# LFY1998/IPDM-PyTorch

Measured on AMD Instinct MI355X. Metric: CT slices/s (full proj+img partial-diffusion sample), higher is better.
Workload: dtype f32

## Files before the change

ipdm-pytorch_amd/csrc/common.h:

```cpp
#pragma once
#include <hip/hip_runtime.h>
#include <cstdarg>
#include <cstdio>
#include <cstring>
#include <string>
#include <vector>
#include "../../include/ipdm_hip.h"

namespace ipdm {

void set_error(const char *fmt, ...);

#define IPDM_HIP_CHECK(expr)                                                                   \
    do {                                                                                       \
        hipError_t e_ = (expr);                                                                \
        if (e_ != hipSuccess) {                                                                \
            ipdm::set_error("%s failed: %s (%s:%d)", #expr, hipGetErrorString(e_), __FILE__,  \
                            __LINE__);                                                         \
            return IPDM_ERR_HIP;                                                               \
        }                                                                                      \
    } while (0)

#define IPDM_REQUIRE(cond, ...)                   \
    do {                                          \
        if (!(cond)) {                            \
            ipdm::set_error(__VA_ARGS__);         \
            return IPDM_ERR_INVALID;              \
        }                                         \
    } while (0)

#define IPDM_LAUNCH_CHECK() IPDM_HIP_CHECK(hipGetLastError())

static inline int cdiv(long a, long b) { return (int)((a + b - 1) / b); }
static inline size_t align_up(size_t v, size_t a) { return (v + a - 1) / a * a; }

enum Opt {
    OPT_CONV_NO_UP2,
    OPT_CONV_NO_WUP2,
    OPT_CONV_LEGACY, OPT_CONV1X1_LEGACY, OPT_CONVS2_LEGACY,
    OPT_CONV_NO_DIRECT, OPT_DIRECT_NO_PLANAR, OPT_DIRECT_MAX_CIN, OPT_DIRECT_NO_S2, OPT_DIRECT_NO_SKIP_FUSE,
    OPT_CONV_DBG, OPT_CONV_VEC4_STRICT, OPT_CONV_NO_SPLITK, OPT_CONV_NO_WINO, OPT_WINO_V1, OPT_WINO2_MIN_TILES, OPT_CONV1X1_NO_QUARTER, OPT_CONV_NO_PW, OPT_PW_ITEM, OPT_PW_FORCE,
    OPT_CONV_NM,
    OPT_GN_TWO_STAGE, OPT_GN_UNFUSED,
    OPT_UNET_TRANSPOSE,
    OPT_ATTN_NO_KVSPLIT, OPT_ATTN_LEGACY, OPT_ATTN_NO_ZSEQ,
    OPT_ART_PER_VIEW,
    OPT_CONV_BF16X3,
    OPT_ATTN_EXACT_F32,
    OPT_ATTN_NO_PRESPLIT,
    OPT_ATTN_NO_PIPELINE,
    OPT_COUNT
};
int opt(Opt o);
bool opt_per_call(int o);
const char *opt_name(int o);
void opt_snapshot(int (&dst)[OPT_COUNT]);
int opt_changed_since(const int (&rec)[OPT_COUNT]);
std::vector<int> opt_per_call_values();

int ensure_dynamic_lds(const void *kernel, size_t bytes);
int device_cu_count();

int unet_io_channels(const ipdm_unet *net, int *cin, int *cout);

__device__ inline double wave_sum(double v)
{
#pragma unroll
    for (int o = 32; o > 0; o >>= 1) v += __shfl_down(v, o, 64);
    return v;
}
__device__ inline float wave_sum(float v)
{
#pragma unroll
    for (int o = 32; o > 0; o >>= 1) v += __shfl_down(v, o, 64);
    return v;
}
__device__ inline float wave_max(float v)
{
#pragma unroll
    for (int o = 32; o > 0; o >>= 1) v = fmaxf(v, __shfl_down(v, o, 64));
    return v;
}

}
```

ipdm-pytorch_amd/csrc/common.hip:

```cpp
#include <cctype>
#include <cstdlib>
#include <mutex>
#include <strings.h>
#include <set>
#include <utility>
#include "common.h"

namespace ipdm {
static thread_local char g_err[512] = "";
void set_error(const char *fmt, ...)
{
    va_list ap;
    va_start(ap, fmt);
    vsnprintf(g_err, sizeof(g_err), fmt, ap);
    va_end(ap);
}

namespace {
std::mutex g_attr_mu;
std::set<std::pair<const void *, int>> g_attr_done;
int g_cus[64];
}

namespace {
struct OptDef { const char *name; int def; bool per_call; int lo = 0, hi = 1; };
const OptDef g_opt_def[OPT_COUNT] = {
    {"conv_no_up2", 0, true},
    {"conv_no_wup2", 0, true},
    {"conv_legacy", 0, false}, {"conv1x1_legacy", 0, false}, {"convs2_legacy", 0, false},
    {"conv_no_direct", 0, false}, {"direct_no_planar", 0, false},
    {"direct_max_cin", 160, false, 0, 160},
    {"direct_no_s2", 0, false}, {"direct_no_skip_fuse", 0, true},
    {"conv_dbg", 0, true, 0, 0x3ff}, {"conv_vec4_strict", 0, false}, {"conv_no_splitk", 0, false},
    {"conv_no_wino", 0, true}, {"wino_v1", 0, true}, {"wino2_min_tiles", 192, true, 0, 1 << 24},
    {"conv1x1_no_quarter", 0, true}, {"conv_no_pw", 0, true}, {"pw_item", 0, true, 0, 2}, {"pw_force", 0, true}, {"conv_nm", 0, true, 0, 2},
    {"gn_two_stage", 0, true}, {"gn_unfused", 0, true},
    {"unet_transpose", -1, true, -1, 1},
    {"attn_no_kvsplit", 0, false}, {"attn_legacy", 0, false}, {"attn_no_zseq", 0, true},
    {"art_per_view", 0, true},
    {"conv_bf16x3", 0, true},
    {"attn_exact_f32", 0, true},
    {"attn_no_presplit", 0, true},
    {"attn_no_pipeline", 0, true},
};
bool opt_value_ok(int i, int v)
{
    return v >= g_opt_def[i].lo && v <= g_opt_def[i].hi;
}
std::mutex g_opt_mu;
int g_opt_val[OPT_COUNT];
bool g_opt_init = false;

void opt_init_locked()
{
    if (g_opt_init) return;
    for (int i = 0; i < OPT_COUNT; ++i) {
        char env[64] = "IPDM_";
        size_t n = 5;
        for (const char *c = g_opt_def[i].name; *c && n + 1 < sizeof(env); ++c) env[n++] = (char)toupper((unsigned char)*c);
        env[n] = 0;
        const char *e = getenv(env);
        g_opt_val[i] = g_opt_def[i].def;
        if (e) {
            char *end = nullptr;
            const long v = strtol(e, &end, 10);
            const int want = (end != e) ? (int)v : 1;
            if (opt_value_ok(i, want)) g_opt_val[i] = want;
            else fprintf(stderr, "libipdm_hip: %s=%s is outside the option's range [%d, %d]: ignored\n", env, e, g_opt_def[i].lo, g_opt_def[i].hi);
        }
    }
    g_opt_init = true;
}
}

int opt(Opt o)
{
    std::lock_guard<std::mutex> lk(g_opt_mu);
    opt_init_locked();
    return g_opt_val[o];
}
bool opt_per_call(int o) { return g_opt_def[o].per_call; }
const char *opt_name(int o) { return g_opt_def[o].name; }
void opt_snapshot(int (&dst)[OPT_COUNT])
{
    std::lock_guard<std::mutex> lk(g_opt_mu);
    opt_init_locked();
    for (int i = 0; i < OPT_COUNT; ++i) dst[i] = g_opt_val[i];
}
std::vector<int> opt_per_call_values()
{
    std::lock_guard<std::mutex> lk(g_opt_mu);
    opt_init_locked();
    std::vector<int> v;
    for (int i = 0; i < OPT_COUNT; ++i)
        if (g_opt_def[i].per_call) v.push_back(g_opt_val[i]);
    return v;
}
int opt_changed_since(const int (&rec)[OPT_COUNT])
{
    std::lock_guard<std::mutex> lk(g_opt_mu);
    opt_init_locked();
    for (int i = 0; i < OPT_COUNT; ++i)
        if (!g_opt_def[i].per_call && g_opt_val[i] != rec[i]) return i;
    return -1;
}
static int opt_find(const char *name)
{
    if (!name) return -1;
    if (!strncmp(name, "IPDM_", 5) || !strncmp(name, "ipdm_", 5)) name += 5;
    for (int i = 0; i < OPT_COUNT; ++i)
        if (!strcasecmp(name, g_opt_def[i].name)) return i;
    return -1;
}

int ensure_dynamic_lds(const void *kernel, size_t bytes)
{
    int dev = 0;
    IPDM_HIP_CHECK(hipGetDevice(&dev));
    std::lock_guard<std::mutex> lk(g_attr_mu);
    if (g_attr_done.count({kernel, dev})) return IPDM_OK;
    IPDM_HIP_CHECK(hipFuncSetAttribute(kernel, hipFuncAttributeMaxDynamicSharedMemorySize, (int)bytes));
    g_attr_done.insert({kernel, dev});
    return IPDM_OK;
}

int device_cu_count()
{
    int dev = 0, v = 0;
    if (hipGetDevice(&dev) != hipSuccess || dev < 0 || dev >= 64) return 256;
    std::lock_guard<std::mutex> lk(g_attr_mu);
    if (!g_cus[dev])
        g_cus[dev] = (hipDeviceGetAttribute(&v, hipDeviceAttributeMultiprocessorCount, dev) == hipSuccess && v > 0) ? v : 256;
    return g_cus[dev];
}
}

extern "C" const char *ipdm_last_error(void) { return ipdm::g_err; }
extern "C" int ipdm_abi_version(void) { return IPDM_ABI_VERSION; }

extern "C" int ipdm_set_option(const char *name, int value)
{
    const int i = ipdm::opt_find(name);
    IPDM_REQUIRE(i >= 0, "ipdm_set_option: unknown option '%s'", name ? name : "(null)");
    IPDM_REQUIRE(ipdm::opt_value_ok(i, value), "ipdm_set_option: %s = %d is outside [%d, %d]", ipdm::g_opt_def[i].name, value,
                 ipdm::g_opt_def[i].lo, ipdm::g_opt_def[i].hi);
    std::lock_guard<std::mutex> lk(ipdm::g_opt_mu);
    ipdm::opt_init_locked();
    ipdm::g_opt_val[i] = value;
    return IPDM_OK;
}

extern "C" int ipdm_get_option(const char *name, int *value)
{
    const int i = ipdm::opt_find(name);
    IPDM_REQUIRE(i >= 0 && value, "ipdm_get_option: unknown option '%s'", name ? name : "(null)");
    *value = ipdm::opt((ipdm::Opt)i);
    return IPDM_OK;
}
```

ipdm-pytorch_amd/csrc/conv_direct.hip:

```cpp
#include <cstdlib>
#include <type_traits>
#include "common.h"
#include "unet_kernels.h"

using namespace ipdm;

typedef float f32x2 __attribute__((ext_vector_type(2)));
typedef float f32x4 __attribute__((ext_vector_type(4)));

namespace {

inline double direct_bytes(const ConvArgs &a)
{
    return 4.0 * a.B * ((double)(a.C1 + a.C2 + (a.sk_w ? a.sk_C1 + a.sk_C2 : 0)) * a.Hs * a.Ws + (double)a.Cout * a.Ho * a.Wo * (a.res ? 2 : 1));
}

inline bool direct_compute_bound(const ConvArgs &a) { return a.C1 + a.C2 >= 64; }
inline double direct_flops(const ConvArgs &a, int taps)
{
    return 2.0 * a.B * a.Ho * a.Wo * a.Cout * ((double)(a.C1 + a.C2) * taps + (a.sk_w ? a.sk_C1 + a.sk_C2 : 0));
}
inline int direct_class(const ConvArgs &a) { return direct_compute_bound(a) ? 6 : 4; }
inline double direct_work(const ConvArgs &a, int taps) { return direct_compute_bound(a) ? direct_flops(a, taps) : direct_bytes(a); }

constexpr int DT_W = 64, DT_H = 16;

struct DTile { int bx, by, n; };
__device__ inline DTile direct_tile()
{
    const int gx = gridDim.x, gy = gridDim.y;
    const int total = gx * gy * gridDim.z;
    const int L = blockIdx.x + gx * (blockIdx.y + gy * blockIdx.z);
    const int xcd = L & 7, idx = L >> 3, q = total >> 3, r = total & 7;
    const int t = xcd * q + min(xcd, r) + idx;
    DTile d;
    d.bx = t % gx;
    const int rest = t / gx;
    d.by = rest % gy;
    d.n = rest / gy;
    return d;
}
constexpr int DIN_P1 = 68;

#define IPDM_DPP_F(v, ctrl) __builtin_bit_cast(float, __builtin_amdgcn_update_dpp(0, __builtin_bit_cast(int, (v)), (ctrl), 0xf, 0xf, false))
__device__ inline float sum_lanes_row(float x)
{
    x += IPDM_DPP_F(x, 0x121);
    x += IPDM_DPP_F(x, 0x122);
    x += IPDM_DPP_F(x, 0x124);
    x += IPDM_DPP_F(x, 0x128);
    return x;
}
#undef IPDM_DPP_F

constexpr int DOOB = 0x7fffffff;
__device__ inline float dload(__amdgpu_buffer_rsrc_t r, int voff, int soff)
{
    return __builtin_bit_cast(float, __builtin_amdgcn_raw_buffer_load_b32(r, voff, soff, 0));
}

template <int CO>
__device__ inline void direct_epilogue(const ConvArgs &a, f32x2 (&acc)[4][CO / 2], int n, int ox0, int oy0, int tx, int ty, float *in_lds)
{
    const int tid = threadIdx.x;
    const int oy = oy0 + ty, ox = ox0 + tx * 4;
    const bool in_img = oy < a.Ho && ox < a.Wo;
    const size_t out_plane = (size_t)a.Ho * a.Wo;
    const bool vec = (a.Wo & 3) == 0;
    const bool full_tile = oy0 + DT_H <= a.Ho && ox0 + DT_W <= a.Wo;
    float *st = in_lds;
    if (a.stats) __syncthreads();
#pragma unroll
    for (int co = 0; co < CO; ++co) {
        if (co < a.Cout) {
            const float b = a.bias ? a.bias[co] : 0.0f;
            const size_t o = ((size_t)n * a.Cout + co) * out_plane + (size_t)oy * a.Wo + ox;
            f32x4 v = {acc[0][co / 2][co & 1] + b, acc[1][co / 2][co & 1] + b, acc[2][co / 2][co & 1] + b, acc[3][co / 2][co & 1] + b};
            if (in_img) {
                if (vec) {
                    if (a.res) v += *reinterpret_cast<const f32x4 *>(a.res + o);
                    *reinterpret_cast<f32x4 *>(a.out + o) = v;
                } else {
#pragma unroll
                    for (int p = 0; p < 4; ++p)
                        if (ox + p < a.Wo) {
                            v[p] += a.res ? a.res[o + p] : 0.0f;
                            a.out[o + p] = v[p];
                        }
                }
            }
            if (a.stats) {
                if (!full_tile) {
#pragma unroll
                    for (int p = 0; p < 4; ++p) v[p] = (in_img && ox + p < a.Wo) ? v[p] : 0.0f;
                }
                st[(2 * co) * 256 + tid] = (v[0] + v[1]) + (v[2] + v[3]);
                st[(2 * co + 1) * 256 + tid] = fmaf(v[3], v[3], fmaf(v[2], v[2], fmaf(v[1], v[1], v[0] * v[0])));
            }
        }
    }
    if (a.stats) {
        __syncthreads();
        const int j = tid & 15;
#pragma unroll
        for (int k = tid >> 4; k < 2 * CO; k += 16) {
            if ((k >> 1) < a.Cout) {
                const f32x4 *src = reinterpret_cast<const f32x4 *>(st + k * 256 + j * 16);
                const f32x4 p0 = src[0], p1 = src[1], p2 = src[2], p3 = src[3];
                float s = (((p0[0] + p0[1]) + (p0[2] + p0[3])) + ((p1[0] + p1[1]) + (p1[2] + p1[3]))) +
                          (((p2[0] + p2[1]) + (p2[2] + p2[3])) + ((p3[0] + p3[1]) + (p3[2] + p3[3])));
                s = sum_lanes_row(s);
                if (j == 0) {
                    const int row = (oy0 / DT_H) * gridDim.x + ox0 / DT_W;
                    a.stats[(((size_t)n * a.stats_rows + row) * a.Cout + (k >> 1)) * 2 + (k & 1)] = s;
                }
            }
        }
    }
}

template <int CO, int KS, int DKC, bool PLANAR, int STRIDE = 1, int SKIP = 0>
__global__ void __launch_bounds__(256, (STRIDE == 2 ? (CO <= 8 ? 4 : 3) : (CO <= 4 ? 6 : (CO <= 8 ? 5 : 3)))) conv_direct_kernel(ConvArgs a)
{
    static_assert(SKIP == 0 || (KS == 3 && STRIDE == 1 && !PLANAR), "conv_direct: the fused shortcut rides on a 3x3 stride-1 NCHW layer");
    constexpr int DIN_H = (DT_H - 1) * STRIDE + KS, DIN_W = (DT_W - 1) * STRIDE + KS, DIN_P = STRIDE == 1 ? DIN_P1 : 132;
    constexpr int DIN_CH = DIN_H * DIN_P, TAPS = KS * KS, PAD = KS / 2;
    static_assert(STRIDE == 1 || (KS == 3 && !PLANAR), "conv_direct: stride 2 is the 3x3 Downsample");
    __shared__ __attribute__((aligned(16))) float in_lds[DKC * DIN_CH];
    typedef const __attribute__((address_space(4))) float cfloat;
    cfloat *wk = (cfloat *)(unsigned long long)a.w;
    cfloat *gsc = (cfloat *)(unsigned long long)a.gn_scale, *gsh = (cfloat *)(unsigned long long)a.gn_shift;
    const int tid = threadIdx.x;
    const int tx = tid & 15, ty = tid >> 4;
    const DTile dt = direct_tile();
    const int n = dt.n;
    const int ox0 = dt.bx * DT_W, oy0 = dt.by * DT_H;
    const int Ctot = a.C1 + a.C2;
    const int src_plane = a.Hs * a.Ws;

    f32x2 acc[4][CO / 2];
#pragma unroll
    for (int p = 0; p < 4; ++p)
#pragma unroll
        for (int c = 0; c < CO / 2; ++c) acc[p][c] = f32x2{0.0f, 0.0f};

    constexpr int NSP = (DIN_H * DIN_W + 255) / 256;
    int sp_src[NSP], sp_srcp[NSP], sp_dst[NSP];
    bool sp_ok[NSP];
#pragma unroll
    for (int j = 0; j < NSP; ++j) {
        const int e = tid + j * 256;
        const int r = e / DIN_W, c = e % DIN_W;
        const int iy = oy0 * STRIDE - PAD + r, ix = ox0 * STRIDE - PAD + c;
        sp_ok[j] = e < DIN_H * DIN_W && iy >= 0 && iy < a.H && ix >= 0 && ix < a.W;
        int sy = min(max(iy, 0), a.H - 1), sx = min(max(ix, 0), a.W - 1);
        if (a.upsample) {
            sy = min((int)floorf((float)sy * a.scale_y), a.Hs - 1);
            sx = min((int)floorf((float)sx * a.scale_x), a.Ws - 1);
        }
        sp_src[j] = e < DIN_H * DIN_W ? (sy * a.Ws + sx) * 4 : DOOB;
        sp_srcp[j] = !(PLANAR || SKIP == 2) ? sp_src[j]
                   : (e < DIN_H * DIN_W ? ((((sy & 1) * 2 + (sx & 1)) * (a.Hs >> 1) + (sy >> 1)) * (a.Ws >> 1) + (sx >> 1)) * 4 : DOOB);
        sp_dst[j] = e < DIN_H * DIN_W ? r * DIN_P + c : -1;
    }
    const int plane_bytes = src_plane * 4;
    const __amdgpu_buffer_rsrc_t rsrc1 = __builtin_amdgcn_make_buffer_rsrc((void *)(a.x1 + (size_t)n * a.C1 * src_plane), 0, a.C1 * plane_bytes, 0x00020000);
    const __amdgpu_buffer_rsrc_t rsrc2 = __builtin_amdgcn_make_buffer_rsrc((void *)(a.x2 ? a.x2 + (size_t)n * a.C2 * src_plane : a.x1), 0, a.x2 ? a.C2 * plane_bytes : 0, 0x00020000);

    auto run_chunks = [&](auto sk_tag) __attribute__((always_inline)) {
    constexpr bool SK = decltype(sk_tag)::value;
    const int C1v = SK ? a.sk_C1 : a.C1, Ctotv = SK ? a.sk_C1 + a.sk_C2 : Ctot;
    const int actv = SK ? 0 : a.act;
    const __amdgpu_buffer_rsrc_t rsA = SK ? __builtin_amdgcn_make_buffer_rsrc((void *)(a.sk_x1 + (size_t)n * a.sk_C1 * src_plane), 0, a.sk_C1 * plane_bytes, 0x00020000) : rsrc1;
    const __amdgpu_buffer_rsrc_t rsB = SK ? __builtin_amdgcn_make_buffer_rsrc((void *)(a.sk_x2 ? a.sk_x2 + (size_t)n * a.sk_C2 * src_plane : a.sk_x1), 0,
                                                                               a.sk_x2 ? a.sk_C2 * plane_bytes : 0, 0x00020000) : rsrc2;
    constexpr bool PL = SK ? SKIP == 2 : PLANAR;
    cfloat *wkv = SK ? (cfloat *)(unsigned long long)a.sk_w : wk;
    const int cpadv = SK ? a.sk_cout_pad : a.cout_pad;
    for (int c0 = 0; c0 < Ctotv; c0 += DKC) {
        const int kc = min(DKC, Ctotv - c0);
        __syncthreads();
        float raw[DKC][NSP];
#pragma unroll
        for (int c = 0; c < DKC; ++c) {
            const int cg = min(c0 + c, Ctotv - 1);
            const bool from1 = cg < C1v;
            const __amdgpu_buffer_rsrc_t r = from1 ? rsA : rsB;
            const int so = (from1 ? cg : cg - C1v) * plane_bytes;
#pragma unroll
            for (int j = 0; j < NSP; ++j) raw[c][j] = dload(r, PL && from1 ? sp_srcp[j] : sp_src[j], so);
        }
#pragma unroll
        for (int c = 0; c < DKC; ++c) {
            if (c < kc) {
                float sc = 1.0f, sh = 0.0f;
                if (actv) { sc = gsc[(size_t)n * Ctot + c0 + c]; sh = gsh[(size_t)n * Ctot + c0 + c]; }
#pragma unroll
                for (int j = 0; j < NSP; ++j) {
                    float v = raw[c][j];
                    if (actv) {
                        v = v * sc + sh;
                        if (actv == 2) v = v * __builtin_amdgcn_rcpf(1.0f + __builtin_amdgcn_exp2f(-1.4426950408889634f * v));
                    }
                    if (sp_dst[j] >= 0) in_lds[c * DIN_CH + sp_dst[j]] = sp_ok[j] ? v : 0.0f;
                }
            }
        }
        __syncthreads();
        for (int c = 0; c < kc; ++c) {
            const float *ip = in_lds + c * DIN_CH + ty * STRIDE * DIN_P + tx * 4 * STRIDE;
#pragma unroll
            for (int ky = 0; ky < KS; ++ky) {
                if (SK && ky != 1) continue;
                const f32x4 lo = *reinterpret_cast<const f32x4 *>(ip + ky * DIN_P);
                f32x2 hi = {0.0f, 0.0f};
                if (KS > 1 && STRIDE == 1) hi = *reinterpret_cast<const f32x2 *>(ip + ky * DIN_P + 4);
                f32x4 mid = {0.0f, 0.0f, 0.0f, 0.0f};
                float last = 0.0f;
                if (STRIDE == 2) { mid = *reinterpret_cast<const f32x4 *>(ip + ky * DIN_P + 4); last = ip[ky * DIN_P + 8]; }
                const float iv[9] = {lo[0], lo[1], lo[2], lo[3], STRIDE == 1 ? hi[0] : mid[0], STRIDE == 1 ? hi[1] : mid[1], mid[2], mid[3], last};
#pragma unroll
                for (int kx = 0; kx < KS; ++kx) {
                    if (SK && kx != 1) continue;
                    cfloat *wp = wkv + (SK ? (size_t)(c0 + c) : (size_t)(c0 + c) * TAPS + ky * KS + kx) * cpadv;
                    f32x2 wv[CO / 2];
#pragma unroll
                    for (int q = 0; q < CO / 2; ++q) wv[q] = f32x2{wp[2 * q], wp[2 * q + 1]};
#pragma unroll
                    for (int p = 0; p < 4; ++p)
#pragma unroll
                        for (int q = 0; q < CO / 2; ++q) acc[p][q] += wv[q] * iv[p * STRIDE + kx];
                }
            }
        }
    }

    };
    run_chunks(std::false_type{});
    if (SKIP) run_chunks(std::true_type{});

    static_assert(2 * CO * 256 <= DKC * DIN_CH, "conv_direct: statistics staging does not fit the input tile area");
    direct_epilogue<CO>(a, acc, n, ox0, oy0, tx, ty, in_lds);
}

template <int CO, int DKC>
__global__ void __launch_bounds__(256, (CO <= 8 ? 5 : 3)) conv_direct_up2_kernel(ConvArgs a)
{
    constexpr int SH = DT_H / 2 + 2, SW = DT_W / 2 + 2, SP = 36, SCH = SH * SP;
    constexpr int LDS_FLOATS = (DKC * SCH > 2 * CO * 256) ? DKC * SCH : 2 * CO * 256;
    __shared__ __attribute__((aligned(16))) float in_lds[LDS_FLOATS];
    typedef const __attribute__((address_space(4))) float cfloat;
    cfloat *wk = (cfloat *)(unsigned long long)a.w_up2;
    const int tid = threadIdx.x, wave = tid >> 6, lane = tid & 63;
    const int tx = lane & 15;
    const int ty = (wave >> 1) * 8 + (lane >> 4) * 2 + (wave & 1);
    const int par_a = __builtin_amdgcn_readfirstlane(wave & 1);
    const DTile dt = direct_tile();
    const int n = dt.n;
    const int ox0 = dt.bx * DT_W, oy0 = dt.by * DT_H;
    const int sx0 = (ox0 >> 1) - 1, sy0 = (oy0 >> 1) - 1;
    const int Cin = a.C1, src_plane = a.Hs * a.Ws, plane_bytes = src_plane * 4;
    const int cin_pad = (Cin + 7) / 8 * 8;

    f32x2 acc[4][CO / 2];
#pragma unroll
    for (int p = 0; p < 4; ++p)
#pragma unroll
        for (int c = 0; c < CO / 2; ++c) acc[p][c] = f32x2{0.0f, 0.0f};

    constexpr int NSP = (SH * SW + 255) / 256;
    int sp_src[NSP], sp_dst[NSP];
#pragma unroll
    for (int j = 0; j < NSP; ++j) {
        const int e = tid + j * 256;
        const int r = e / SW, c = e % SW;
        const int sy = sy0 + r, sx = sx0 + c;
        const bool ok = e < SH * SW && sy >= 0 && sy < a.Hs && sx >= 0 && sx < a.Ws;
        sp_src[j] = ok ? (sy * a.Ws + sx) * 4 : DOOB;
        sp_dst[j] = e < SH * SW ? r * SP + c : -1;
    }
    const __amdgpu_buffer_rsrc_t rsrc = __builtin_amdgcn_make_buffer_rsrc((void *)(a.x1 + (size_t)n * Cin * src_plane), 0, Cin * plane_bytes, 0x00020000);

    for (int c0 = 0; c0 < Cin; c0 += DKC) {
        const int kc = min(DKC, Cin - c0);
        __syncthreads();
        float raw[DKC][NSP];
#pragma unroll
        for (int c = 0; c < DKC; ++c) {
            const int so = min(c0 + c, Cin - 1) * plane_bytes;
#pragma unroll
            for (int j = 0; j < NSP; ++j) raw[c][j] = dload(rsrc, sp_src[j], so);
        }
#pragma unroll
        for (int c = 0; c < DKC; ++c)
#pragma unroll
            for (int j = 0; j < NSP; ++j)
                if (sp_dst[j] >= 0) in_lds[c * SCH + sp_dst[j]] = raw[c][j];
        __syncthreads();
        for (int c = 0; c < kc; ++c) {
            const float *ip = in_lds + c * SCH + ((ty >> 1) + par_a) * SP + tx * 2;
#pragma unroll
            for (int i = 0; i < 2; ++i) {
                const f32x2 lo = *reinterpret_cast<const f32x2 *>(ip + i * SP), hi = *reinterpret_cast<const f32x2 *>(ip + i * SP + 2);
                const float iv[4] = {lo[0], lo[1], hi[0], hi[1]};
#pragma unroll
                for (int b = 0; b < 2; ++b)
#pragma unroll
                    for (int j = 0; j < 2; ++j) {
                        cfloat *wp = wk + (((size_t)(par_a * 2 + b) * cin_pad + c0 + c) * 4 + i * 2 + j) * a.cout_pad;
                        f32x2 wv[CO / 2];
#pragma unroll
                        for (int q = 0; q < CO / 2; ++q) wv[q] = f32x2{wp[2 * q], wp[2 * q + 1]};
#pragma unroll
                        for (int q = 0; q < CO / 2; ++q) {
                            acc[b][q] += wv[q] * iv[j + b];
                            acc[2 + b][q] += wv[q] * iv[1 + j + b];
                        }
                    }
            }
        }
    }
    direct_epilogue<CO>(a, acc, n, ox0, oy0, tx, ty, in_lds);
}

template <int CO>
int launch_direct_s2(const ConvArgs &a, hipStream_t st)
{
    dim3 grid(cdiv(a.Wo, DT_W), cdiv(a.Ho, DT_H), a.B);
    const bool prof = prof_enabled();
    if (prof) prof_before(direct_class(a), st);
    hipLaunchKernelGGL((conv_direct_kernel<CO, 3, 2, false, 2>), grid, dim3(256), 0, st, a);
    if (prof) prof_after(direct_class(a), direct_work(a, 9), st);
    IPDM_LAUNCH_CHECK();
    return IPDM_OK;
}

template <int CO, int KS>
int launch_direct(const ConvArgs &a, hipStream_t st)
{
    dim3 grid(cdiv(a.Wo, DT_W), cdiv(a.Ho, DT_H), a.B);
    const bool prof = prof_enabled();
    if (prof) prof_before(direct_class(a), st);
    if constexpr (KS == 3 && CO >= 8) {
        if (a.sk_w) {
            if (a.sk_planar) hipLaunchKernelGGL((conv_direct_kernel<CO, KS, (CO <= 8 ? 4 : 8), false, 1, 2>), grid, dim3(256), 0, st, a);
            else hipLaunchKernelGGL((conv_direct_kernel<CO, KS, (CO <= 8 ? 4 : 8), false, 1, 1>), grid, dim3(256), 0, st, a);
            if (prof) prof_after(direct_class(a), direct_work(a, KS * KS), st);
            IPDM_LAUNCH_CHECK();
            return IPDM_OK;
        }
    }
    if (a.x1_planar) hipLaunchKernelGGL((conv_direct_kernel<CO, KS, (CO <= 8 ? 4 : 8), true>), grid, dim3(256), 0, st, a);
    else hipLaunchKernelGGL((conv_direct_kernel<CO, KS, (CO <= 8 ? 4 : 8), false>), grid, dim3(256), 0, st, a);
    if (prof) prof_after(direct_class(a), direct_work(a, KS * KS), st);
    IPDM_LAUNCH_CHECK();
    return IPDM_OK;
}

}

namespace ipdm {

bool conv_direct_eligible(const ConvArgs &a)
{
    const int max_cin = opt(OPT_DIRECT_MAX_CIN);
    const int cin = a.C1 + a.C2;
    const bool no_s2 = opt(OPT_DIRECT_NO_S2) != 0;
    if (a.stride == 2)
        return !no_s2 && a.ksize == 3 && a.Cout <= 16 && cin <= 32 && !a.upsample && !a.x1_planar && a.w_interleave == 0 && a.cout_pad >= 16;
    return (a.ksize == 3 || a.ksize == 1) && a.stride == 1 && a.Cout <= 16 && (cin <= max_cin || (a.Cout <= 4 && cin <= 128)) && a.w_interleave == 0 &&
           a.cout_pad >= 16;
}

bool conv_direct_up2_eligible(const ConvArgs &a)
{
    const bool off = opt(OPT_CONV_NO_UP2) != 0;
    return !off && a.w_up2 && a.w_interleave == 0 && a.ksize == 3 && a.stride == 1 && a.C2 == 0 && a.act == 0 && !a.res &&
           !a.x1_planar && a.H == 2 * a.Hs && a.W == 2 * a.Ws && a.Ho == a.H && a.Wo == a.W && a.Cout > 4 && a.Cout <= 16 &&
           a.C1 <= 64 && a.cout_pad >= 16;
}

int conv_direct_stats_rows(const ConvArgs &a) { return cdiv(a.Wo, DT_W) * cdiv(a.Ho, DT_H); }

bool conv_direct_skip_ok(const ConvArgs &a)
{
    if (opt(OPT_CONV_NO_DIRECT) || opt(OPT_DIRECT_NO_SKIP_FUSE)) return false;
    return conv_direct_eligible(a) && a.ksize == 3 && a.stride == 1 && !a.upsample && !a.x1_planar && !a.C2 && !a.res && a.Cout > 4 && a.Cout <= 16 &&
           a.sk_C1 > 0 && a.sk_C1 + a.sk_C2 <= opt(OPT_DIRECT_MAX_CIN) && a.sk_cout_pad >= 16 && !conv_direct_up2_eligible(a);
}

int conv2d_direct_launch(const ConvArgs &a, hipStream_t st)
{
    IPDM_REQUIRE(conv_direct_eligible(a), "conv2d_direct: layer not eligible");
    IPDM_REQUIRE(!a.stats || a.stats_rows == conv_direct_stats_rows(a), "conv2d: statistics rows %d != %d", a.stats_rows,
                 conv_direct_stats_rows(a));
    IPDM_REQUIRE(!a.x1_planar || (!a.upsample && !(a.Hs & 1) && !(a.Ws & 1)), "conv2d: parity-planar input of odd size %dx%d", a.Hs, a.Ws);
    IPDM_REQUIRE((long)a.C1 * a.Hs * a.Ws < (1L << 29) && (long)(a.C2 + 1) * a.Hs * a.Ws < (1L << 29),
                 "conv2d: per-sample tensor exceeds the 2 GiB buffer-addressing range");
    IPDM_REQUIRE(!a.sk_w || conv_direct_skip_ok(a), "conv2d: this layer cannot carry a fused shortcut");
    IPDM_REQUIRE(!a.sk_w || ((long)a.sk_C1 * a.Hs * a.Ws < (1L << 29) && (long)(a.sk_C2 + 1) * a.Hs * a.Ws < (1L << 29)),
                 "conv2d: the fused shortcut's source exceeds the 2 GiB buffer-addressing range");
    IPDM_REQUIRE(!a.sk_w || !a.sk_planar || (!(a.Hs & 1) && !(a.Ws & 1)), "conv2d: parity-planar shortcut source of odd size %dx%d", a.Hs, a.Ws);
    if (a.stride == 2) {
        if (a.Cout <= 4) return launch_direct_s2<4>(a, st);
        if (a.Cout <= 8) return launch_direct_s2<8>(a, st);
        return launch_direct_s2<16>(a, st);
    }
    if (conv_direct_up2_eligible(a)) {
        dim3 grid(cdiv(a.Wo, DT_W), cdiv(a.Ho, DT_H), a.B);
        const bool prof = prof_enabled();
        if (prof) prof_before(4, st);
        if (a.Cout <= 8) hipLaunchKernelGGL((conv_direct_up2_kernel<8, 8>), grid, dim3(256), 0, st, a);
        else hipLaunchKernelGGL((conv_direct_up2_kernel<16, 8>), grid, dim3(256), 0, st, a);
        if (prof) prof_after(4, direct_bytes(a), st);
        IPDM_LAUNCH_CHECK();
        return IPDM_OK;
    }
    if (a.ksize == 1) {
        if (a.Cout <= 4) return launch_direct<4, 1>(a, st);
        if (a.Cout <= 8) return launch_direct<8, 1>(a, st);
        return launch_direct<16, 1>(a, st);
    }
    if (a.Cout <= 4) return launch_direct<4, 3>(a, st);
    if (a.Cout <= 8) return launch_direct<8, 3>(a, st);
    return launch_direct<16, 3>(a, st);
}

}
```

Before: 2.205.

## Stream fused 1x1 shortcut from global memory and raise direct-conv occupancy

```diff
diff --git a/ipdm-pytorch_amd/csrc/common.h b/ipdm-pytorch_amd/csrc/common.h
--- a/ipdm-pytorch_amd/csrc/common.h
+++ b/ipdm-pytorch_amd/csrc/common.h
@@ -49,6 +49,7 @@
     OPT_ATTN_EXACT_F32,
     OPT_ATTN_NO_PRESPLIT,
     OPT_ATTN_NO_PIPELINE,
+    OPT_DIRECT_NO_WALK,
     OPT_COUNT
 };
 int opt(Opt o);
diff --git a/ipdm-pytorch_amd/csrc/common.hip b/ipdm-pytorch_amd/csrc/common.hip
--- a/ipdm-pytorch_amd/csrc/common.hip
+++ b/ipdm-pytorch_amd/csrc/common.hip
@@ -42,6 +42,7 @@
     {"attn_exact_f32", 0, true},
     {"attn_no_presplit", 0, true},
     {"attn_no_pipeline", 0, true},
+    {"direct_no_walk", 0, true},
 };
 bool opt_value_ok(int i, int v)
 {
diff --git a/ipdm-pytorch_amd/csrc/conv_direct.hip b/ipdm-pytorch_amd/csrc/conv_direct.hip
--- a/ipdm-pytorch_amd/csrc/conv_direct.hip
+++ b/ipdm-pytorch_amd/csrc/conv_direct.hip
@@ -59,6 +59,15 @@
     return __builtin_bit_cast(float, __builtin_amdgcn_raw_buffer_load_b32(r, voff, soff, 0));
 }
 
+__device__ inline f32x4 dload4(__amdgpu_buffer_rsrc_t r, int voff, int soff)
+{
+    return __builtin_bit_cast(f32x4, __builtin_amdgcn_raw_buffer_load_b128(r, voff, soff, 0));
+}
+__device__ inline f32x2 dload2(__amdgpu_buffer_rsrc_t r, int voff, int soff)
+{
+    return __builtin_bit_cast(f32x2, __builtin_amdgcn_raw_buffer_load_b64(r, voff, soff, 0));
+}
+
 template <int CO>
 __device__ inline void direct_epilogue(const ConvArgs &a, f32x2 (&acc)[4][CO / 2], int n, int ox0, int oy0, int tx, int ty, float *in_lds)
 {
@@ -119,8 +128,8 @@
     }
 }
 
-template <int CO, int KS, int DKC, bool PLANAR, int STRIDE = 1, int SKIP = 0>
-__global__ void __launch_bounds__(256, (STRIDE == 2 ? (CO <= 8 ? 4 : 3) : (CO <= 4 ? 6 : (CO <= 8 ? 5 : 3)))) conv_direct_kernel(ConvArgs a)
+template <int CO, int KS, int DKC, bool PLANAR, int STRIDE = 1, int SKIP = 0, bool OLD = false>
+__global__ void __launch_bounds__(256, (STRIDE == 2 ? (CO <= 8 ? 4 : 3) : (CO <= 4 ? 6 : (CO <= 8 ? (KS == 3 && !SKIP && !PLANAR && !OLD ? 7 : 5) : (SKIP && !OLD ? 4 : 3))))) conv_direct_kernel(ConvArgs a)
 {
     static_assert(SKIP == 0 || (KS == 3 && STRIDE == 1 && !PLANAR), "conv_direct: the fused shortcut rides on a 3x3 stride-1 NCHW layer");
     constexpr int DIN_H = (DT_H - 1) * STRIDE + KS, DIN_W = (DT_W - 1) * STRIDE + KS, DIN_P = STRIDE == 1 ? DIN_P1 : 132;
@@ -159,7 +168,7 @@
             sx = min((int)floorf((float)sx * a.scale_x), a.Ws - 1);
         }
         sp_src[j] = e < DIN_H * DIN_W ? (sy * a.Ws + sx) * 4 : DOOB;
-        sp_srcp[j] = !(PLANAR || SKIP == 2) ? sp_src[j]
+        sp_srcp[j] = !(PLANAR || (SKIP == 2 && OLD)) ? sp_src[j]
                    : (e < DIN_H * DIN_W ? ((((sy & 1) * 2 + (sx & 1)) * (a.Hs >> 1) + (sy >> 1)) * (a.Ws >> 1) + (sx >> 1)) * 4 : DOOB);
         sp_dst[j] = e < DIN_H * DIN_W ? r * DIN_P + c : -1;
     }
@@ -190,21 +199,46 @@
 #pragma unroll
             for (int j = 0; j < NSP; ++j) raw[c][j] = dload(r, PL && from1 ? sp_srcp[j] : sp_src[j], so);
         }
-#pragma unroll
-        for (int c = 0; c < DKC; ++c) {
-            if (c < kc) {
-                float sc = 1.0f, sh = 0.0f;
-                if (actv) { sc = gsc[(size_t)n * Ctot + c0 + c]; sh = gsh[(size_t)n * Ctot + c0 + c]; }
-#pragma unroll
-                for (int j = 0; j < NSP; ++j) {
-                    float v = raw[c][j];
-                    if (actv) {
-                        v = v * sc + sh;
-                        if (actv == 2) v = v * __builtin_amdgcn_rcpf(1.0f + __builtin_amdgcn_exp2f(-1.4426950408889634f * v));
+        auto stage = [&](auto act_tag) __attribute__((always_inline)) {
+            constexpr int ACT = decltype(act_tag)::value;
+#pragma unroll
+            for (int c = 0; c < DKC; ++c) {
+                if (c < kc) {
+                    float sc = 1.0f, sh = 0.0f;
+                    if (ACT) { sc = gsc[(size_t)n * Ctot + c0 + c]; sh = gsh[(size_t)n * Ctot + c0 + c]; }
+#pragma unroll
+                    for (int j = 0; j < NSP; ++j) {
+                        float v = raw[c][j];
+                        if (ACT) {
+                            v = v * sc + sh;
+                            if (ACT == 2) v = v * __builtin_amdgcn_rcpf(1.0f + __builtin_amdgcn_exp2f(-1.4426950408889634f * v));
+                        }
+                        if (j < NSP - 1 || sp_dst[j] >= 0) in_lds[c * DIN_CH + sp_dst[j]] = sp_ok[j] ? v : 0.0f;
                     }
-                    if (sp_dst[j] >= 0) in_lds[c * DIN_CH + sp_dst[j]] = sp_ok[j] ? v : 0.0f;
-                }
-            }
+                }
+            }
+        };
+        if constexpr (OLD || PLANAR || CO > 8 || KS != 3) {
+#pragma unroll
+            for (int c = 0; c < DKC; ++c) {
+                if (c < kc) {
+                    float sc = 1.0f, sh = 0.0f;
+                    if (actv) { sc = gsc[(size_t)n * Ctot + c0 + c]; sh = gsh[(size_t)n * Ctot + c0 + c]; }
+#pragma unroll
+                    for (int j = 0; j < NSP; ++j) {
+                        float v = raw[c][j];
+                        if (actv) {
+                            v = v * sc + sh;
+                            if (actv == 2) v = v * __builtin_amdgcn_rcpf(1.0f + __builtin_amdgcn_exp2f(-1.4426950408889634f * v));
+                        }
+                        if (sp_dst[j] >= 0) in_lds[c * DIN_CH + sp_dst[j]] = sp_ok[j] ? v : 0.0f;
+                    }
+                }
+            }
+        } else {
+            if (actv == 2) stage(std::integral_constant<int, 2>{});
+            else if (actv == 1) stage(std::integral_constant<int, 1>{});
+            else stage(std::integral_constant<int, 0>{});
         }
         __syncthreads();
         for (int c = 0; c < kc; ++c) {
@@ -237,7 +271,71 @@
 
     };
     run_chunks(std::false_type{});
-    if (SKIP) run_chunks(std::true_type{});
+    if constexpr (SKIP != 0 && OLD) run_chunks(std::true_type{});
+
+    if constexpr (SKIP != 0 && !OLD) {
+        constexpr int G = CO <= 8 ? 2 : 4;
+        const int C1v = a.sk_C1, Ctotv = a.sk_C1 + a.sk_C2;
+        const __amdgpu_buffer_rsrc_t rsA = __builtin_amdgcn_make_buffer_rsrc((void *)(a.sk_x1 + (size_t)n * a.sk_C1 * src_plane), 0, a.sk_C1 * plane_bytes, 0x00020000);
+        const __amdgpu_buffer_rsrc_t rsB = __builtin_amdgcn_make_buffer_rsrc((void *)(a.sk_x2 ? a.sk_x2 + (size_t)n * a.sk_C2 * src_plane : a.sk_x1), 0,
+                                                                               a.sk_x2 ? a.sk_C2 * plane_bytes : 0, 0x00020000);
+        cfloat *wkv = (cfloat *)(unsigned long long)a.sk_w;
+        const int cpadv = a.sk_cout_pad;
+        const int oy = oy0 + ty, ox = ox0 + tx * 4;
+        const bool in_img = oy < a.H && ox < a.W;
+        const int o_lin = in_img ? (oy * a.Ws + ox) * 4 : 0;
+        const int o_pl = in_img ? (((oy & 1) * 2 * (a.Hs >> 1) + (oy >> 1)) * (a.Ws >> 1) + (ox >> 1)) * 4 : 0;
+        const int quarter_bytes = (a.Hs >> 1) * (a.Ws >> 1) * 4;
+        const bool vec = (a.Ws & 3) == 0;
+        const int wl = in_img ? a.W - 1 - ox : 0;
+        {
+            auto load_group = [&](int c0, f32x4 (&x)[G]) __attribute__((always_inline)) {
+#pragma unroll
+                for (int c = 0; c < G; ++c) {
+                    const int cg = min(c0 + c, Ctotv - 1);
+                    const bool from1 = cg < C1v;
+                    const __amdgpu_buffer_rsrc_t r = from1 ? rsA : rsB;
+                    const int so = (from1 ? cg : cg - C1v) * plane_bytes;
+                    if (SKIP == 2 && from1) {
+                        if (vec) {
+                            const f32x2 ev = dload2(r, o_pl, so), od = dload2(r, o_pl, so + quarter_bytes);
+                            x[c] = f32x4{ev[0], od[0], ev[1], od[1]};
+                        } else {
+                            const int dq = wl >= 2 ? 4 : 0;
+                            x[c] = f32x4{dload(r, o_pl, so), dload(r, o_pl, so + quarter_bytes), dload(r, o_pl + dq, so), dload(r, o_pl + dq, so + quarter_bytes)};
+                        }
+                    } else {
+                        if (vec) x[c] = dload4(r, o_lin, so);
+                        else x[c] = f32x4{dload(r, o_lin, so), dload(r, o_lin + min(1, wl) * 4, so), dload(r, o_lin + min(2, wl) * 4, so), dload(r, o_lin + min(3, wl) * 4, so)};
+                    }
+                }
+            };
+            auto fma_group = [&](int c0, const f32x4 (&x)[G]) __attribute__((always_inline)) {
+#pragma unroll
+                for (int c = 0; c < G; ++c) {
+                    if (c0 + c < Ctotv) {
+                        cfloat *wp = wkv + (size_t)(c0 + c) * cpadv;
+                        f32x2 wv[CO / 2];
+#pragma unroll
+                        for (int q = 0; q < CO / 2; ++q) wv[q] = f32x2{wp[2 * q], wp[2 * q + 1]};
+#pragma unroll
+                        for (int p = 0; p < 4; ++p)
+#pragma unroll
+                            for (int q = 0; q < CO / 2; ++q) acc[p][q] += wv[q] * x[c][p];
+                    }
+                }
+            };
+            f32x4 xa[G], xb[G];
+            load_group(0, xa);
+#pragma unroll 1
+            for (int c0 = 0; c0 < Ctotv; c0 += 2 * G) {
+                if (c0 + G < Ctotv) load_group(c0 + G, xb);
+                fma_group(c0, xa);
+                if (c0 + 2 * G < Ctotv) load_group(c0 + 2 * G, xa);
+                fma_group(c0 + G, xb);
+            }
+        }
+    }
 
     static_assert(2 * CO * 256 <= DKC * DIN_CH, "conv_direct: statistics staging does not fit the input tile area");
     direct_epilogue<CO>(a, acc, n, ox0, oy0, tx, ty, in_lds);
@@ -329,7 +427,8 @@
     dim3 grid(cdiv(a.Wo, DT_W), cdiv(a.Ho, DT_H), a.B);
     const bool prof = prof_enabled();
     if (prof) prof_before(direct_class(a), st);
-    hipLaunchKernelGGL((conv_direct_kernel<CO, 3, 2, false, 2>), grid, dim3(256), 0, st, a);
+    if (CO > 8 || opt(OPT_DIRECT_NO_WALK)) hipLaunchKernelGGL((conv_direct_kernel<CO, 3, 2, false, 2, 0, true>), grid, dim3(256), 0, st, a);
+    else if constexpr (CO <= 8) hipLaunchKernelGGL((conv_direct_kernel<CO, 3, 2, false, 2>), grid, dim3(256), 0, st, a);
     if (prof) prof_after(direct_class(a), direct_work(a, 9), st);
     IPDM_LAUNCH_CHECK();
     return IPDM_OK;
@@ -341,17 +440,25 @@
     dim3 grid(cdiv(a.Wo, DT_W), cdiv(a.Ho, DT_H), a.B);
     const bool prof = prof_enabled();
     if (prof) prof_before(direct_class(a), st);
+    const bool old = opt(OPT_DIRECT_NO_WALK) != 0 || (CO > 8 && !(a.sk_w && a.sk_planar));
     if constexpr (KS == 3 && CO >= 8) {
         if (a.sk_w) {
-            if (a.sk_planar) hipLaunchKernelGGL((conv_direct_kernel<CO, KS, (CO <= 8 ? 4 : 8), false, 1, 2>), grid, dim3(256), 0, st, a);
-            else hipLaunchKernelGGL((conv_direct_kernel<CO, KS, (CO <= 8 ? 4 : 8), false, 1, 1>), grid, dim3(256), 0, st, a);
+            constexpr int DKC = CO <= 8 ? 4 : 8;
+            if (old) {
+                if (a.sk_planar) hipLaunchKernelGGL((conv_direct_kernel<CO, KS, DKC, false, 1, 2, true>), grid, dim3(256), 0, st, a);
+                else hipLaunchKernelGGL((conv_direct_kernel<CO, KS, DKC, false, 1, 1, true>), grid, dim3(256), 0, st, a);
+            } else {
+                if (a.sk_planar) hipLaunchKernelGGL((conv_direct_kernel<CO, KS, DKC, false, 1, 2>), grid, dim3(256), 0, st, a);
+                else if constexpr (CO <= 8) hipLaunchKernelGGL((conv_direct_kernel<CO, KS, DKC, false, 1, 1>), grid, dim3(256), 0, st, a);
+            }
             if (prof) prof_after(direct_class(a), direct_work(a, KS * KS), st);
             IPDM_LAUNCH_CHECK();
             return IPDM_OK;
         }
     }
     if (a.x1_planar) hipLaunchKernelGGL((conv_direct_kernel<CO, KS, (CO <= 8 ? 4 : 8), true>), grid, dim3(256), 0, st, a);
-    else hipLaunchKernelGGL((conv_direct_kernel<CO, KS, (CO <= 8 ? 4 : 8), false>), grid, dim3(256), 0, st, a);
+    else if (old) hipLaunchKernelGGL((conv_direct_kernel<CO, KS, (CO <= 8 ? 4 : 8), false, 1, 0, true>), grid, dim3(256), 0, st, a);
+    else if constexpr (CO <= 8) hipLaunchKernelGGL((conv_direct_kernel<CO, KS, (CO <= 8 ? 4 : 8), false>), grid, dim3(256), 0, st, a);
     if (prof) prof_after(direct_class(a), direct_work(a, KS * KS), st);
     IPDM_LAUNCH_CHECK();
     return IPDM_OK;
```

Result: no change. 2.212, median of 6 (+0.3%).
